# hall-lab/svtyper

Hardware: AMD Instinct MI355X
Metric: breakpoints genotyped/sec (higher is better)
Workload: dtype f64

## Files before the change

include/svtyper_reads.h:

```cpp
#ifndef SVTYPER_READS_H
#define SVTYPER_READS_H

#include <stdint.h>

#include "svtyper_hip.h"

#ifdef __cplusplus
extern "C" {
#endif

typedef struct svt_bam svt_bam;

int svt_bam_open(const char* path, svt_bam** out);
void svt_bam_close(svt_bam* bam);

int32_t svt_bam_n_references(const svt_bam* bam);
const char* svt_bam_reference_name(const svt_bam* bam, int32_t tid);
int64_t svt_bam_reference_length(const svt_bam* bam, int32_t tid);
int32_t svt_bam_tid(const svt_bam* bam, const char* name);
const char* svt_bam_header_text(const svt_bam* bam);

typedef struct svt_fetch_unit {
    int32_t tid_a, lo_a, hi_a;
    int32_t tid_b, lo_b, hi_b;
// ... 43 lines not shown
#define SVT_WALK_SA_CAP 6
#define SVT_WALK_NO_RG 7
#define SVT_WALK_UNKNOWN_RG 8
#define SVT_WALK_MALFORMED 9
#define SVT_WALK_MAPQ 10
#define SVT_WALK_N_REASONS 11

#define SVT_WALK_CAP_READS 0
#define SVT_WALK_CAP_NAME 1
#define SVT_WALK_CAP_CIGAR 2
#define SVT_WALK_CAP_SA_ENTRIES 3
#define SVT_WALK_CAP_SA_BYTES 4
#define SVT_WALK_CAP_RECORD 5
#define SVT_WALK_CAP_READS_LDS 6
uint32_t svt_evidence_walk_capacity(int which);

int svt_bam_evidence_walk_host(const svt_bam* bam, const svt_summarise_args* args, const svt_evidence_params* geometry,
                               svt_evidence* out, uint8_t* out_of_envelope, uint32_t* kept_reads);

typedef struct svt_evidence_device_stats {
    uint64_t n_units;
    uint64_t reads_walked;
    uint64_t units_skipped;
    uint64_t units_host;
    uint64_t units_host_by_reason[SVT_WALK_N_REASONS];
    uint64_t n_records;
    uint64_t bytes_uploaded;
    double host_arena_s;
    double upload_s;
    double device_walk_s;
// ... 100 lines not shown
```

svtyper_amd/csrc/svt_entry_evidence.h:

```cpp

static int run_inflate_kernel(const uint8_t* d_src, uint64_t src_len, const inf::Member* d_members, uint64_t n, uint8_t* d_dst, uint64_t dst_len,
                              uint32_t* d_status, std::vector<uint32_t>& status, hipStream_t s)
{
    status.assign(n, 0);
    constexpr uint64_t kGrid = 1u << 30;
    for (uint64_t at = 0; at < n; at += kGrid) {
        const uint64_t m = std::min(kGrid, n - at);
        hipLaunchKernelGGL(svt_inflate_kernel, dim3((unsigned)m), dim3(kInflateBlock), 0, s, d_src, src_len, d_members + at, (uint32_t)m, d_dst, dst_len,
                           d_status + at);
        HIP_TRY(hipGetLastError());
    }
    if (n) HIP_TRY(hipMemcpyAsync(status.data(), d_status, n * sizeof(uint32_t), hipMemcpyDeviceToHost, s));
    HIP_TRY(hipStreamSynchronize(s));
    return SVT_OK;
}

static thread_local svt_evidence_deep_stats g_deep_stats{};

struct EvidenceRoute {
    svt_evidence_inflate_stats* inflate_stats = nullptr;
    bool count_host_blocks = false;
    bool device_inflate() const { return inflate_stats != nullptr; }
};

struct EvidenceCall : CallStream {
    const svt_bam* const bam;
    const svt_summarise_args* const args;
    const svt_evidence_params* const geometry;
    const svt_evidence_batch* const header;
    const int device;
    const unsigned flags;
    const EvidenceRoute route;
    svt_evidence_device_stats& S;
    svt_evidence_deep_stats& DS = g_deep_stats;
    const uint64_t n = args->n_units;
    Pooled d_arena{device}, d_records{device}, d_compressed{device};
    DevScratch d_members, d_member_status;
    DevScratch d_ranges, d_units, d_windows, d_bps, d_rgs, d_refs, d_blob, d_flank, d_status, d_rows, d_reads, d_off, d_src, d_src_off, d_dst_off;
    DevScratch d_deep_unit, d_deep_status, d_deep_rows, d_deep_workspace;

    ew::Arena arena;
    ew::OpenPlan plan;
    EvidenceArgs a{};
    EvidenceDeepArgs da{};
    static constexpr size_t kLds = sizeof(ew::UnitScratch);
    std::vector<uint32_t> status, rows, reads;
    std::vector<uint32_t> deep_unit;
    uint32_t n_deep = 0, deep_grid = 0;
    std::vector<uint64_t> host_ids, host_counts;
    std::vector<svt_record> host_records;
    std::vector<uint8_t> host_skipped;
    std::vector<uint64_t> rec_offset;
    std::vector<svt_unit> units;
// ... 37 lines not shown
                svt_evidence_inflate_stats& I = *route.inflate_stats;
                SVT_TRY(d_compressed.get(plan.compressed_bytes + 8));
                for (const auto& sp : plan.spans) SVT_TRY(st.copy(static_cast<uint8_t*>(d_compressed.p) + sp.at, plan.file + sp.file_off, sp.bytes));
                SVT_TRY(upload(d_members, plan.members, st));
                SVT_TRY(d_member_status.alloc(plan.members.size() * sizeof(uint32_t)));
                SVT_TRY(st.finish());
                I.compressed_upload_s = since(t0);
                const auto t_kernel = now();
                std::vector<uint32_t> member_status;
                SVT_TRY(run_inflate_kernel(static_cast<const uint8_t*>(d_compressed.p), plan.compressed_bytes, d_members.as<inf::Member>(), plan.members.size(),
                                           static_cast<uint8_t*>(d_arena.p), plan.arena_bytes, d_member_status.as<uint32_t>(), member_status, s));
                I.inflate_kernel_s = since(t_kernel);
                I.blocks_failed = ew::apply_member_status(plan, member_status, arena);
            } else SVT_TRY(st.copy(d_arena.p, arena.bytes.data(), arena.bytes.size()));
            SVT_TRY(upload(d_ranges, arena.ranges, st));
            SVT_TRY(upload(d_units, arena.units, st));
            SVT_TRY(d_windows.alloc(n * sizeof(svt_fetch_unit)));
            SVT_TRY(st.copy(d_windows.p, args->windows, n * sizeof(svt_fetch_unit)));
            SVT_TRY(d_bps.alloc(n * sizeof(svt_breakpoint)));
            SVT_TRY(st.copy(d_bps.p, args->breakpoints, n * sizeof(svt_breakpoint)));
            SVT_TRY(upload(d_rgs, arena.rgs, st));
            SVT_TRY(upload(d_refs, arena.refs, st));
            SVT_TRY(upload(d_blob, arena.blob, st));
            SVT_TRY(upload(d_flank, flank, st));
            SVT_TRY(st.finish());
            S.bytes_uploaded = (route.device_inflate() ? plan.compressed_bytes + plan.members.size() * sizeof(inf::Member) : arena.bytes.size()) + arena.ranges.size() * sizeof(ew::Range) + n * (sizeof(ew::UnitRanges) + sizeof(svt_fetch_unit) + sizeof(svt_breakpoint)) + arena.blob.size();
        }
        SVT_TRY(d_status.alloc(n * sizeof(uint32_t)));
        SVT_TRY(d_rows.alloc(n * sizeof(uint32_t)));
        SVT_TRY(d_reads.alloc(n * sizeof(uint32_t)));
        SVT_TRY(d_off.alloc((n + 1) * sizeof(uint64_t)));
        HIP_TRY(hipStreamSynchronize(s));
        S.upload_s = since(t0);
        return SVT_OK;
    }
    int bind_arguments()
    {
        a.P = arena.params(args, geometry);
        a.P.arena = static_cast<const uint8_t*>(d_arena.p);
        a.P.ranges = d_ranges.as<ew::Range>();
        a.P.units = d_units.as<ew::UnitRanges>();
        a.P.windows = d_windows.as<svt_fetch_unit>();
        a.P.bps = d_bps.as<svt_breakpoint>();
        a.P.rgs = d_rgs.as<ew::NameRef>();
        a.P.refs = d_refs.as<ew::NameRef>();
        a.P.blob = d_blob.as<uint8_t>();
        a.P.lib_flank = d_flank.as<double>();
        a.n_units = (uint32_t)n;
        a.status = d_status.as<uint32_t>();
        a.n_rows = d_rows.as<uint32_t>();
        a.n_reads = d_reads.as<uint32_t>();
        a.rec_offset = d_off.as<uint64_t>();
        a.records = nullptr;
        static_assert(sizeof(ew::UnitScratch) <= 80 * 1024, "two workgroups of the evidence kernel per CU");
        static_assert(sizeof(ew::DeepScratch) <= 64 * 1024, "the deep kernel's static LDS");
// ... 253 lines not shown
```

svtyper_amd/csrc/svt_evidence_arena.h:

```cpp
#ifndef SVT_EVIDENCE_ARENA_H
#define SVT_EVIDENCE_ARENA_H

#include <cstdint>
#include <string>
#include <vector>

#include "svt_evidence_walk.h"
#include "svt_inflate.h"

namespace svt {
namespace ew {

struct Arena {
    std::vector<uint8_t> bytes;
    std::vector<Range> ranges;
    std::vector<UnitRanges> units;
    std::vector<NameRef> rgs, refs;
    std::vector<uint8_t> blob;
    uint64_t records_in_ranges = 0;
    uint64_t blocks = 0;
    double build_s = 0.0;
    bool open_ranges = false;
    Params params(const svt_summarise_args* args, const svt_evidence_params* geometry) const
    {
        Params P{};
        P.arena = bytes.data();
        P.arena_len = bytes.size();
        P.ranges = ranges.data();
        P.units = units.data();
        P.windows = args->windows;
        P.bps = args->breakpoints;
        P.rgs = rgs.data();
        P.refs = refs.data();
        P.blob = blob.data();
        P.lib_flank = geometry->lib_flank;
        P.n_rgs = (uint32_t)rgs.size();
        P.n_refs = (uint32_t)refs.size();
        P.n_libs = geometry->n_libs;
        P.min_aligned = geometry->min_aligned;
        P.split_slop = geometry->split_slop;
        P.count_mode = args->count_mode;
        P.max_reads = args->max_reads;
        P.open_ranges = open_ranges ? 1u : 0u;
        return P;
    }
};

inline bool deep_tier_unit(uint32_t status, uint32_t n_reads) { return status == EW_READS && n_reads <= kMaxReadsDeep; }


int build_arena(const svt_bam* bam, const svt_summarise_args* args, const svt_evidence_params* geometry, Arena& out);

struct OpenPlan {
    struct Span { uint64_t file_off, bytes, at; };
    const uint8_t* file = nullptr;
    uint64_t file_size = 0;
    std::vector<Span> spans;
    uint64_t compressed_bytes = 0;
    uint64_t arena_bytes = 0;
    std::vector<inf::Member> members;
    std::vector<std::pair<uint32_t, uint32_t>> range_members;
    double index_s = 0.0;
};

int build_arena_open(const svt_bam* bam, const svt_summarise_args* args, const svt_evidence_params* geometry, Arena& out, OpenPlan& plan);
void inflate_open_host(const OpenPlan& plan, Arena& out, unsigned n_threads, std::vector<uint32_t>& status);
// ... 12 lines not shown
```

svtyper_amd/csrc/svt_evidence_kernel.h:

```cpp
#ifndef SVT_EVIDENCE_KERNEL_H
#define SVT_EVIDENCE_KERNEL_H

#include "svt_evidence_walk.h"

namespace svt {

constexpr int kEvidenceBlock = 256;

struct EvidenceDevCtx {
    static __device__ __forceinline__ uint32_t lane() { return threadIdx.x; }
    static __device__ __forceinline__ uint32_t lanes() { return kEvidenceBlock; }
    static __device__ __forceinline__ void sync() { __syncthreads(); }
};

struct EvidenceArgs {
    ew::Params P;
    uint32_t n_units;
    uint32_t* status;
    uint32_t* n_rows;
    uint32_t* n_reads;
    const uint64_t* rec_offset;
    uint4* records;
};

// ... 64 lines not shown
```

svtyper_amd/csrc/svt_evidence_walk.h:

```cpp
#ifndef SVT_EVIDENCE_WALK_H
#define SVT_EVIDENCE_WALK_H

#include <stdint.h>

#include "../../include/svtyper_reads.h"
#include "svt_geometry_math.h"
#include "svt_record_rules.h"

namespace svt {
namespace ew {

using namespace rr;

constexpr uint32_t kMaxReads = 1024;
constexpr uint32_t kMaxReadsDeep = 16384;
constexpr uint32_t kSortTile = 2048;
constexpr uint32_t kMaxName = 128;
constexpr uint32_t kMaxCigar = 256;
constexpr uint32_t kMaxSaEntries = 8;
constexpr uint32_t kMaxSaBytes = 1024;
constexpr uint32_t kMaxRecord = 1u << 16;
constexpr uint32_t kBatch = 256;

enum : uint32_t {
    EW_OK = 0,
    EW_SKIPPED = 1,
    EW_RANGE = 2,
    EW_READS = 3,
    EW_NAME = 4,
    EW_CIGAR = 5,
    EW_SA_CAP = 6,
    EW_NO_RG = 7,
    EW_UNKNOWN_RG = 8,
    EW_MALFORMED = 9,
    EW_MAPQ = 10,
    EW_N_STATUS = 11
};

struct Range { uint32_t begin, end; };
struct UnitRanges { uint32_t first; uint16_t n[2]; uint32_t preset; };
struct NameRef { uint32_t off, len; int32_t value; };

struct Params {
    const uint8_t* arena;
    uint64_t arena_len;
    const Range* ranges;
    const UnitRanges* units;
    const svt_fetch_unit* windows;
    const svt_breakpoint* bps;
    const NameRef* rgs;
    const NameRef* refs;
    const uint8_t* blob;
    const double* lib_flank;
    uint32_t n_rgs, n_refs, n_libs;
    int32_t min_aligned, split_slop;
    int32_t count_mode;
    int64_t max_reads;
    uint32_t open_ranges;
};

struct ReadSum {
// ... 59 lines not shown
constexpr uint64_t kDeepSliceBytes = (uint64_t)kMaxReadsDeep * (sizeof(ReadSum) + sizeof(uint64_t) + 3 * sizeof(uint32_t));
static_assert(sizeof(ReadSum) == 52 && kDeepSliceBytes == 1179648, "1 179 648 bytes per slice");
SVT_HD Tables<uint32_t> deep_tables(uint8_t* slice)
{
    Tables<uint32_t> T;
    T.reads = reinterpret_cast<ReadSum*>(slice);
    T.key = reinterpret_cast<uint64_t*>(slice + (uint64_t)kMaxReadsDeep * sizeof(ReadSum));
    T.order = reinterpret_cast<uint32_t*>(T.key + kMaxReadsDeep);
    T.rows = T.order + kMaxReadsDeep;
    T.rowoff = T.rows + kMaxReadsDeep;
    T.cap = kMaxReadsDeep;
    return T;
}

struct HostCtx {
    static SVT_HD uint32_t lane() { return 0; }
    static SVT_HD uint32_t lanes() { return 1; }
    static SVT_HD void sync() {}
};

SVT_HD bool bytes_eq(const uint8_t* a, const uint8_t* b, uint32_t n)
{
    for (uint32_t i = 0; i < n; ++i) if (a[i] != b[i]) return false;
    return true;
}
SVT_HD int name_cmp(const uint8_t* a, uint32_t na, const uint8_t* b, uint32_t nb)
{
    const uint32_t n = na < nb ? na : nb;
    for (uint32_t i = 0; i < n; ++i) if (a[i] != b[i]) return a[i] < b[i] ? -1 : 1;
    return na < nb ? -1 : na > nb ? 1 : 0;
// ... 48 lines not shown
    if (r.tid >= 0 && (uint32_t)r.tid < P.n_refs) {
        const NameRef& nr = P.refs[r.tid];
        same_chrom = nr.len == fl[0] && bytes_eq(P.blob + nr.off, sa + fo[0], fl[0]);
    }
    const bool b_rev = fl[2] == 1 && sa[fo[2]] == '-';
    const Piece pa = {r.tid, r.pos, r.end, a_rev, query_pos(a, a_rev)};
    const Piece pb = {b_at < 0 ? -3 : b_at, mate_pos1 - 1, mate_pos1 - 1 + b.ref, b_rev, query_pos(b, b_rev)};
    bool self_left;
    if (!split_valid(pa, pb, same_chrom, left_clipped(a), self_left)) return EW_OK;
    rs.o_tid = pb.tid; rs.o_start = clip32(pb.start); rs.o_end = clip32(pb.end); rs.o_mapq = (uint8_t)mate_mapq;
    rs.bits |= (uint8_t)(RS_SPLIT | (b_rev ? RS_O_REV : 0) | (self_left ? RS_SELF_LEFT : 0));
    return EW_OK;
}

struct Eval { bool ovl, counted, keep; uint32_t early, late; };
SVT_HD void eval_record(const Params& P, const uint8_t* d, uint32_t size, uint32_t arena_off, int32_t wtid, int64_t lo, int64_t hi,
                        int64_t near_a, int64_t near_b, Eval& e, ReadSum& rs)
{
    e.ovl = e.counted = e.keep = false;
    e.early = e.late = EW_OK;
    Core r;
    if (!decode_core(d, size, r) || r.l_seq < 0 || r.tid != wtid || (int64_t)r.pos >= hi) { e.ovl = true; e.early = EW_RANGE; return; }
    int64_t rend = r.end;
    if (r.n_cigar == 0 || rend <= r.pos) rend = (int64_t)r.pos + 1;
    if (!(rend > lo)) return;
    e.ovl = true;
    e.counted = !(r.flag & (0x4 | 0x100 | 0x200 | 0x400));
    if (r.flag & (0x4 | 0x400)) return;
    Tags t;
    tags_begin(t);
    uint32_t tags_at = r.tags_off;
    const bool tags_ok = walk_tags(d, size, tags_at, false, t) == TAGS_END;
    if (!t.have_rg) { e.early = EW_NO_RG; return; }
    const int32_t at = find_name(P.rgs, P.n_rgs, P.blob, d + t.rg_off, t.rg_len);
    if (at < 0) { e.early = EW_UNKNOWN_RG; return; }
    const int32_t lib = P.rgs[at].value;
    if (lib < 0) return;
    e.keep = true;
    if (!tags_ok) { e.late = EW_MALFORMED; return; }
    if ((uint32_t)lib >= P.n_libs || lib > 0xffff) { e.late = EW_UNKNOWN_RG; return; }
    const uint32_t name_len = r.l_name ? r.l_name - 1 : 0;
// ... 9 lines not shown
    rs.flag = (uint16_t)r.flag;
    rs.lib = (uint16_t)lib;
    rs.mapq = (uint8_t)r.mapq;
    rs.o_mapq = 0;
    rs.bits = (uint8_t)((r.flag & 0x10) ? RS_REV : 0);
    if (r.flag & (0x100 | 0x800)) return;
    Intervals iv;
    aligned_intervals(d + 32 + r.l_name, r.n_cigar, r.pos, near_a, near_b, iv);
    rs.iv_s[0] = clip32(iv.s[0]); rs.iv_e[0] = clip32(iv.e[0]);
    rs.iv_s[1] = clip32(iv.s[1]); rs.iv_e[1] = clip32(iv.e[1]);
    rs.bits |= (uint8_t)iv.n;
    e.late = split_candidate(P, d, r, t, rs);
}

template <class X, class SC>
SVT_HD void gather_window(const Params& P, SC& S, const Tables<typename SC::Idx>& T, const Range* ranges, uint32_t n_ranges, int32_t wtid, int64_t lo, int64_t hi,
                          int64_t near_a, int64_t near_b)
{
    const uint32_t lane = X::lane(), lanes = X::lanes();
    const bool mode1 = P.count_mode == 1 && P.max_reads >= 0, mode0 = P.count_mode == 0 && P.max_reads >= 0;
    typedef Tables<typename SC::Idx> Tb;
    if (lo < 0) lo = 0;
    X::sync();
    if (lane == 0) { S.n_ovl = 0; S.n_counted = 0; S.window_done = 0; }
    for (uint32_t ri = 0; ri < n_ranges; ++ri) {
        const Range rg = ranges[ri];
        X::sync();
        if (S.window_done) break;
        if (lane == 0) {
            S.pos = rg.begin;
            S.range_done = 0;
            if (rg.end < rg.begin || (uint64_t)rg.end > P.arena_len) { if (S.status == EW_OK) S.status = EW_RANGE; }
        }
        X::sync();
        while (S.status == EW_OK && !S.range_done) {
            X::sync();
            if (lane == 0) {
                uint32_t nb = 0, pos = S.pos;
                while (nb < kBatch && pos < rg.end) {
                    if ((uint64_t)pos + 4 > rg.end) { S.status = EW_RANGE; break; }
                    const uint32_t size = ld32(P.arena + pos);
                    if (size < 32 || size > kMaxRecord || (uint64_t)pos + 4 + size > rg.end) { S.status = EW_RANGE; break; }
                    if (P.open_ranges && ((int32_t)ld32(P.arena + pos + 4) != wtid || (int64_t)(int32_t)ld32(P.arena + pos + 8) >= hi)) { S.window_done = 1; break; }
                    S.b.off[nb] = pos + 4;
                    S.b.size[nb] = size;
                    ++nb;
                    pos += 4 + size;
                }
                S.nb = nb;
                S.pos = pos;
                S.n_walked += nb;
                if (pos >= rg.end || nb == 0 || S.window_done) S.range_done = 1;
            }
            X::sync();
            if (S.status != EW_OK) break;
            const uint32_t nb = S.nb;
            for (uint32_t k = lane; k < nb; k += lanes) {
                Eval e;
                eval_record(P, P.arena + S.b.off[k], S.b.size[k], S.b.off[k], wtid, lo, hi, near_a, near_b, e, S.b.rs[k]);
                S.b.ovl[k] = e.ovl;
                S.b.counted[k] = e.counted;
                S.b.keep[k] = e.keep;
                S.b.ev[k] = (uint8_t)(e.early | (e.late << 4));
            }
            X::sync();
            if (lane == 0) {
                uint32_t n_ovl = S.n_ovl, n_counted = S.n_counted, n_reads = S.n_reads, st = EW_OK;
                for (uint32_t k = 0; k < nb && st == EW_OK; ++k) {
                    S.b.slot[k] = Tb::kNoSlot;
                    if (!S.b.ovl[k]) continue;
                    const int64_t i = (int64_t)n_ovl++;
                    const uint32_t early = S.b.ev[k] & 0xF, late = S.b.ev[k] >> 4;
                    if (early == EW_RANGE) { st = EW_RANGE; break; }
                    if (mode1 && S.b.counted[k] && (int64_t)++n_counted > P.max_reads) { st = EW_SKIPPED; break; }
                    if (early != EW_OK) { st = early; break; }
                    if (!S.b.keep[k]) continue;
                    if (mode0 && i > P.max_reads) { st = EW_SKIPPED; break; }
                    if (late != EW_OK) { st = late; break; }
                    if (n_reads < T.cap) S.b.slot[k] = (typename SC::Idx)n_reads;
                    ++n_reads;
                }
                S.n_ovl = n_ovl;
                S.n_counted = n_counted;
                S.n_reads = n_reads;
                if (st != EW_OK) S.status = st;
            }
            X::sync();
            if (S.status != EW_OK) break;
            for (uint32_t k = lane; k < nb; k += lanes)
                if (S.b.slot[k] != Tb::kNoSlot) T.reads[S.b.slot[k]] = S.b.rs[k];
            X::sync();
        }
        X::sync();
        if (S.status != EW_OK) return;
    }
}

SVT_HD ReadS absent_read() { ReadS r; r.tid = -1; r.start = r.end = r.iv0s = r.iv1s = r.iv0e = r.iv1e = 0; r.mapq = r.flags = r.extra = 0; return r; }
SVT_HD PieceS absent_piece() { PieceS p; p.tid = p.start = p.end = 0; p.mapq = p.flags = 0; return p; }
SVT_HD ReadS read_of_sum(const ReadSum& s)
{
    ReadS r;
    r.tid = s.tid; r.start = s.start; r.end = s.end;
    r.iv0s = s.iv_s[0]; r.iv1s = s.iv_s[1]; r.iv0e = s.iv_e[0]; r.iv1e = s.iv_e[1];
    r.mapq = s.mapq;
// ... 115 lines not shown
        X::sync();
    }
}

template <class X, class SC>
SVT_HD void walk_unit(const Params& P, uint64_t u, SC& S, const Tables<typename SC::Idx>& T, Record4* out)
{
    typedef typename SC::Idx Idx;
    typedef Tables<Idx> Tb;
    const uint32_t lane = X::lane(), lanes = X::lanes();
    const UnitRanges ur = P.units[u];
    const svt_fetch_unit w = P.windows[u];
    const svt_breakpoint bp = P.bps[u];
    if (lane == 0) { S.n_reads = 0; S.n_walked = 0; S.n_rows = 0; S.status = ur.preset; S.lcp = 0; }
    X::sync();
    if (S.status == EW_OK) gather_window<X>(P, S, T, P.ranges + ur.first, ur.n[0], w.tid_a, w.lo_a, w.hi_a, bp.pos_a, bp.pos_b);
    X::sync();
    if (S.status == EW_OK) gather_window<X>(P, S, T, P.ranges + ur.first + ur.n[0], ur.n[1], w.tid_b, w.lo_b, w.hi_b, bp.pos_a, bp.pos_b);
    X::sync();
    if (lane == 0 && S.status == EW_OK && S.n_reads > T.cap) S.status = EW_READS;
    X::sync();
    if (S.status != EW_OK) return;
    const uint32_t n = S.n_reads;
    if (n == 0) return;

    {
        uint32_t lcp = T.reads[0].name_len;
        const uint8_t* a = P.arena + T.reads[0].name_off;
        for (uint32_t k = lane; k < n; k += lanes) {
            const uint8_t* b = P.arena + T.reads[k].name_off;
            const uint32_t m = lcp < T.reads[k].name_len ? lcp : T.reads[k].name_len;
            uint32_t i = 0;
            while (i < m && a[i] == b[i]) ++i;
// ... 102 lines not shown
```

svtyper_amd/csrc/svt_reads.cpp:

```cpp

#include <dlfcn.h>
#include <fcntl.h>
#include <sys/mman.h>
#include <sys/stat.h>
#include <time.h>
#include <unistd.h>
#include <zlib.h>

#include <algorithm>
#include <atomic>
#include <chrono>
#include <condition_variable>
#include <cstdint>
#include <cstdio>
#include <cstdlib>
#include <cstring>
#include <map>
#include <memory>
#include <mutex>
#include <set>
#include <string>
#include <thread>
#include <unordered_map>
#include <vector>
// ... 1016 lines not shown
    if (args->n_units >= 0xFFFFFFF0ull) return fail(SVT_ERR_INVALID, "too many units in one call (< 2^32)");
    return SVT_OK;
}

void arena_names(const svt_bam* bam, const svt_summarise_args* args, Arena& out)
{
    auto add_name = [&](std::vector<NameRef>& tab, const char* p, size_t len, int32_t value) {
        tab.push_back(NameRef{(uint32_t)out.blob.size(), (uint32_t)len, value});
        out.blob.insert(out.blob.end(), p, p + len);
    };
    for (uint32_t i = 0; i < args->n_read_groups; ++i) add_name(out.rgs, args->read_groups[i], std::strlen(args->read_groups[i]), args->read_group_lib[i]);
    for (size_t i = 0; i < bam->ref_names.size(); ++i) add_name(out.refs, bam->ref_names[i].data(), bam->ref_names[i].size(), (int32_t)i);
    out.blob.resize(out.blob.size() + 8, 0);
}

struct RawRange { uint64_t first, last; uint32_t uoff, end_in_last; };
struct UnitRaw { uint64_t at = 0; unsigned worker = 0; uint16_t n[2] = {0, 0}; uint32_t preset = EW_OK; };
struct UnitPlan { std::vector<UnitRaw> units; std::vector<std::vector<RawRange>> ranges; };

enum : unsigned { kChunkRange = 1, kChunkLast = 2, kChunkHost = 4 };

template <typename Worker, typename Route>
int plan_units(const svt_bam* bam, const svt_summarise_args* args, unsigned nt, Route& route, UnitPlan& plan)
{
    const uint64_t n = args->n_units;
    plan.units.assign(n, UnitRaw());
    plan.ranges.assign(nt, std::vector<RawRange>());
    std::atomic<uint64_t> next(0);
    std::atomic<int> first_rc(SVT_OK);
    run_threads(nt, [&](unsigned t) {
        Worker worker(route, t);
// ... 3 lines not shown
            const uint64_t u0 = next.fetch_add(16);
            if (u0 >= n) return;
            for (uint64_t u = u0; u < std::min(n, u0 + 16); ++u) {
                UnitRaw& U = plan.units[u];
                U.at = list.size();
                U.worker = t;
                const svt_fetch_unit& w = args->windows[u];
                const int32_t tids[2] = {w.tid_a, w.tid_b};
                const int64_t los[2] = {w.lo_a, w.lo_b}, his[2] = {w.hi_a, w.hi_b};
                if (args->breakpoints[u].svtype > SVT_SVTYPE_BND) U.preset = EW_RANGE;
                for (int s = 0; s < 2 && U.preset == EW_OK; ++s) {
                    if (tids[s] < 0 || tids[s] >= (int32_t)bam->ref_names.size()) { U.preset = EW_RANGE; break; }
                    const int64_t beg = std::max<int64_t>(los[s], 0), end = his[s];
                    if (end <= beg) continue;
                    for (const auto& c : fetch_chunks(*bam, tids[s], beg, end)) {
                        RawRange r{0, 0, 0, 0};
                        const unsigned got = worker.chunk(tids[s], end, c.first, c.second, r);
                        if ((got & kChunkHost) || ((got & kChunkRange) && U.n[s] == 0xFFFF)) { U.preset = EW_RANGE; break; }
                        if (got & kChunkRange) { list.push_back(r); ++U.n[s]; }
                        if (got & kChunkLast) break;
                    }
                }
                if (U.preset != EW_OK) {
                    list.resize(U.at);
                    U.n[0] = U.n[1] = 0;
                }
            }
        }
    });
    if (first_rc.load() != SVT_OK) return fail(first_rc.load(), "cannot set up the inflate state");
    return SVT_OK;
// ... 8 lines not shown
        for (const RawRange& r : list) needs.push_back(Need{r.first, r.last});
    std::sort(needs.begin(), needs.end(), [](const Need& a, const Need& b) { return a.first < b.first; });
    for (size_t i = 0; i < needs.size();) {
        uint64_t last = needs[i].last;
        size_t j = i + 1;
        while (j < needs.size() && needs[j].first <= last) { last = std::max(last, needs[j].last); ++j; }
        if (const int rc = place(needs[i].first, last)) return rc;
        i = j;
    }
    return SVT_OK;
}

struct Placed { uint64_t at; uint32_t nth; };

void finish_ranges(UnitPlan& plan, const std::unordered_map<uint64_t, Placed>& placed, Arena& out,
                   std::vector<std::pair<uint32_t, uint32_t>>* range_members)
{
    const uint64_t n = plan.units.size();
    out.units.resize(n);
    for (uint64_t u = 0; u < n; ++u) {
        UnitRaw& U = plan.units[u];
        const RawRange* list = plan.ranges[U.worker].data() + U.at;
        const uint64_t nr = (uint64_t)U.n[0] + U.n[1];
        const size_t mark = out.ranges.size();
        for (uint64_t k = 0; k < nr; ++k) {
            const RawRange& r = list[k];
            const auto f = placed.find(r.first), l = placed.find(r.last);
            if (f == placed.end() || l == placed.end()) { U.preset = EW_RANGE; break; }
            const uint64_t begin = f->second.at + r.uoff, end = l->second.at + r.end_in_last;
            if (end > kArenaLimit) { U.preset = EW_RANGE; break; }
            out.ranges.push_back(Range{(uint32_t)std::min(begin, end), (uint32_t)end});
            if (range_members) range_members->emplace_back(f->second.nth, l->second.nth);
        }
        if (U.preset != EW_OK) {
            out.ranges.resize(mark);
            if (range_members) range_members->resize(mark);
            U.n[0] = U.n[1] = 0;
        }
        out.units[u] = UnitRanges{(uint32_t)mark, {U.n[0], U.n[1]}, U.preset};
    }
    out.ranges.push_back(Range{0, 0});
}

struct HostRoute {
    const svt_bam* bam;
    SharedBlocks shared_blocks;
    std::vector<std::vector<std::pair<uint64_t, BlockRef>>> touched;
    std::vector<uint64_t> n_records;
    HostRoute(const svt_bam* b, unsigned nt) : bam(b), touched(nt), n_records(nt, 0) {}
};
struct HostWorker {
    Bgzf z;
    std::vector<uint8_t> buf;
    uint64_t& n_records;
    HostWorker(HostRoute& route, unsigned t) : z(route.bam->file, &route.shared_blocks), n_records(route.n_records[t]) { z.touched = &route.touched[t]; }
    bool ok() const { return z.ok(); }
    unsigned chunk(int32_t tid, int64_t end, uint64_t vbeg, uint64_t vend, RawRange& r)
    {
        unsigned got = 0;
        z.seek(vbeg);
        while (z.tell() < vend) {
            const uint64_t at = z.tell();
            const bool beyond_block = z.offset_in_empty_block();
            uint32_t size = 0;
            const uint8_t* d = next_record(z, buf, size);
            if (!d) {
                if (z.failed() || z.tell() != at) got |= kChunkHost;
                break;
            }
            if ((int32_t)ld32(d) != tid || (int64_t)(int32_t)ld32(d + 4) >= end) { got |= kChunkLast; break; }
            if (!(got & kChunkRange)) {
                r.first = at >> 16;
                r.uoff = (uint32_t)(at & 0xFFFF);
                got |= kChunkRange;
                if (beyond_block) got |= kChunkHost;
            }
            z.last_read(&r.last, &r.end_in_last);
            ++n_records;
        }
        if (z.failed()) got |= kChunkHost;
        return got;
    }
};

struct OpenWorker {
    const OpenPlan& f;
    OpenWorker(OpenPlan& plan, unsigned) : f(plan) {}
    bool ok() const { return true; }
    unsigned chunk(int32_t, int64_t, uint64_t vbeg, uint64_t vend, RawRange& r) const
    {
        if (vend <= vbeg) return 0;
        const uint64_t cb = vbeg >> 16, ce = vend >> 16;
        const uint32_t ub = (uint32_t)(vbeg & 0xFFFF), ue = (uint32_t)(vend & 0xFFFF);
// ... 7 lines not shown
                break;
            }
            if (!inf::member_at(f.file, f.file_size, coff, src, clen, isize, next)) return kChunkHost;
            if (coff == cb && ub > isize) return kChunkHost;
            r.last = coff;
            r.end_in_last = isize;
            if (coff == ce) { r.end_in_last = std::min(ue, isize); break; }
            if (next > ce) return kChunkHost;
            if (next == ce && ue == 0) break;
            coff = next;
        }
        return kChunkRange;
    }
};

}

int build_arena(const svt_bam* bam, const svt_summarise_args* args, const svt_evidence_params* geometry, Arena& out)
{
    if (const int rc = check_arena_args(bam, args, geometry)) return rc;
    const auto t_begin = std::chrono::steady_clock::now();
    out = Arena();
    arena_names(bam, args, out);
    const unsigned nt = arena_threads(args, args->n_units);
    const std::unique_ptr<HostRoute> route(new HostRoute(bam, nt));
    UnitPlan plan;
    if (const int rc = plan_units<HostWorker>(bam, args, nt, *route, plan)) return rc;

    std::unordered_map<uint64_t, BlockRef> blocks;
    for (auto& log : route->touched) {
        for (auto& e : log) blocks.emplace(e.first, e.second);
// ... 14 lines not shown
        }
    });
    out.bytes.resize(std::min<uint64_t>(total, kArenaLimit) + 8);
    {
        std::atomic<size_t> at(0);
        run_threads(std::min<unsigned>(nt, 16u), [&](unsigned) {
            for (;;) {
                const size_t k = at.fetch_add(8);
                if (k >= copies.size()) return;
                for (size_t c = k; c < std::min(copies.size(), k + 8); ++c)
                    if (copies[c].at + copies[c].b->data.size() <= kArenaLimit && !copies[c].b->data.empty())
                        std::memcpy(out.bytes.data() + copies[c].at, copies[c].b->data.data(), copies[c].b->data.size());
            }
        });
    }
    finish_ranges(plan, placed, out, nullptr);
    for (uint64_t c : route->n_records) out.records_in_ranges += c;
    out.blocks = copies.size();
    out.build_s = std::chrono::duration<double>(std::chrono::steady_clock::now() - t_begin).count();
    return SVT_OK;
}

int build_arena_open(const svt_bam* bam, const svt_summarise_args* args, const svt_evidence_params* geometry, Arena& out, OpenPlan& plan)
{
    if (const int rc = check_arena_args(bam, args, geometry)) return rc;
    const auto t_begin = std::chrono::steady_clock::now();
    out = Arena();
    out.open_ranges = true;
    plan = OpenPlan();
    plan.file = bam->file.data;
    plan.file_size = bam->file.size;
// ... 13 lines not shown
                placed[coff] = Placed{total, (uint32_t)plan.members.size()};
                plan.members.push_back(inf::Member{span.at + (src - span.file_off), clen, isize, total});
                span.bytes = next - span.file_off;
            }
            total += isize;
            if (coff == last) break;
            coff = next;
        }
        if (span.bytes) { plan.spans.push_back(span); plan.compressed_bytes += span.bytes; }
        return (int)SVT_OK;
    });
    if (rc) return rc;
    plan.arena_bytes = plan.members.empty() ? 0 : plan.members.back().dst + plan.members.back().isize;
    out.bytes.resize(plan.arena_bytes + 8);
    out.blocks = plan.members.size();
    finish_ranges(units, placed, out, &plan.range_members);
    plan.index_s = out.build_s = std::chrono::duration<double>(std::chrono::steady_clock::now() - t_begin).count();
    return SVT_OK;
}

void inflate_open_host(const OpenPlan& plan, Arena& out, unsigned n_threads, std::vector<uint32_t>& status)
{
    const size_t m = plan.members.size();
    status.assign(m, inf::INF_OK);
    std::atomic<size_t> next(0);
    run_threads(std::max(1u, std::min<unsigned>(n_threads, (unsigned)std::max<size_t>(m, 1))), [&](unsigned) {
        std::unique_ptr<inf::Scratch> S(new inf::Scratch());
        for (;;) {
            const size_t k0 = next.fetch_add(8);
            if (k0 >= m) return;
            for (size_t k = k0; k < std::min(m, k0 + 8); ++k) {
// ... 502 lines not shown
{
    return guarded([&]() -> int {
        if (n && (!status || (!out && out_off && out_off[n]))) return fail(SVT_ERR_INVALID, "null argument");
        std::vector<svt::inf::Member> members(n);
        if (const int rc = svt::ew::bgzf_members(data, len, block_off, n, out_off, members.data())) return rc;
        std::unique_ptr<svt::inf::Scratch> S(new svt::inf::Scratch());
        for (uint64_t k = 0; k < n; ++k) {
            const svt::inf::Member& m = members[k];
            status[k] = m.isize == svt::inf::kNoMember ? (uint32_t)svt::inf::INF_MEMBER
                                                       : svt::inf::inflate_member<svt::inf::HostCtx>(data + m.src, m.clen, out + m.dst, m.isize, *S);
        }
        return SVT_OK;
    });
}

uint32_t svt_evidence_walk_capacity(int which)
{
    switch (which) {
    case SVT_WALK_CAP_READS: return svt::ew::kMaxReadsDeep;
    case SVT_WALK_CAP_READS_LDS: return svt::ew::kMaxReads;
    case SVT_WALK_CAP_NAME: return svt::ew::kMaxName;
    case SVT_WALK_CAP_CIGAR: return svt::ew::kMaxCigar;
    case SVT_WALK_CAP_SA_ENTRIES: return svt::ew::kMaxSaEntries;
    case SVT_WALK_CAP_SA_BYTES: return svt::ew::kMaxSaBytes;
    case SVT_WALK_CAP_RECORD: return svt::ew::kMaxRecord;
    default: return 0;
    }
}

static int svt_bam_scan_library_impl(const svt_bam* bam, uint32_t n_read_groups, const char* const* read_groups, int64_t num_samp,
// ... 489 lines not shown
```

Before: 3.447 billion.

## Parallelise evidence range walk with host-recorded record checkpoints

Result: no change. 3.423 billion (-0.7%).

```diff
diff --git a/include/svtyper_reads.h b/include/svtyper_reads.h
--- a/include/svtyper_reads.h
+++ b/include/svtyper_reads.h
@@ -81,6 +81,7 @@
 #define SVT_WALK_CAP_RECORD 5
 #define SVT_WALK_CAP_READS_LDS 6
 uint32_t svt_evidence_walk_capacity(int which);
+int svt_debug_walk_checkpoints(int on);
 
 int svt_bam_evidence_walk_host(const svt_bam* bam, const svt_summarise_args* args, const svt_evidence_params* geometry,
                                svt_evidence* out, uint8_t* out_of_envelope, uint32_t* kept_reads);
diff --git a/svtyper_amd/csrc/svt_entry_evidence.h b/svtyper_amd/csrc/svt_entry_evidence.h
--- a/svtyper_amd/csrc/svt_entry_evidence.h
+++ b/svtyper_amd/csrc/svt_entry_evidence.h
@@ -36,7 +36,7 @@
     const uint64_t n = args->n_units;
     Pooled d_arena{device}, d_records{device}, d_compressed{device};
     DevScratch d_members, d_member_status;
-    DevScratch d_ranges, d_units, d_windows, d_bps, d_rgs, d_refs, d_blob, d_flank, d_status, d_rows, d_reads, d_off, d_src, d_src_off, d_dst_off;
+    DevScratch d_ranges, d_range_cps, d_checkpoints, d_units, d_windows, d_bps, d_rgs, d_refs, d_blob, d_flank, d_status, d_rows, d_reads, d_off, d_src, d_src_off, d_dst_off;
     DevScratch d_deep_unit, d_deep_status, d_deep_rows, d_deep_workspace;
 
     ew::Arena arena;
@@ -104,6 +104,10 @@
                 I.blocks_failed = ew::apply_member_status(plan, member_status, arena);
             } else SVT_TRY(st.copy(d_arena.p, arena.bytes.data(), arena.bytes.size()));
             SVT_TRY(upload(d_ranges, arena.ranges, st));
+            if (!arena.range_cps.empty()) {
+                SVT_TRY(upload(d_range_cps, arena.range_cps, st));
+                SVT_TRY(upload(d_checkpoints, arena.checkpoints, st));
+            }
             SVT_TRY(upload(d_units, arena.units, st));
             SVT_TRY(d_windows.alloc(n * sizeof(svt_fetch_unit)));
             SVT_TRY(st.copy(d_windows.p, args->windows, n * sizeof(svt_fetch_unit)));
@@ -114,7 +118,7 @@
             SVT_TRY(upload(d_blob, arena.blob, st));
             SVT_TRY(upload(d_flank, flank, st));
             SVT_TRY(st.finish());
-            S.bytes_uploaded = (route.device_inflate() ? plan.compressed_bytes + plan.members.size() * sizeof(inf::Member) : arena.bytes.size()) + arena.ranges.size() * sizeof(ew::Range) + n * (sizeof(ew::UnitRanges) + sizeof(svt_fetch_unit) + sizeof(svt_breakpoint)) + arena.blob.size();
+            S.bytes_uploaded = (route.device_inflate() ? plan.compressed_bytes + plan.members.size() * sizeof(inf::Member) : arena.bytes.size()) + arena.ranges.size() * sizeof(ew::Range) + arena.range_cps.size() * sizeof(ew::RangeCheckpoints) + (arena.range_cps.empty() ? 0 : arena.checkpoints.size() * sizeof(uint32_t)) + n * (sizeof(ew::UnitRanges) + sizeof(svt_fetch_unit) + sizeof(svt_breakpoint)) + arena.blob.size();
         }
         SVT_TRY(d_status.alloc(n * sizeof(uint32_t)));
         SVT_TRY(d_rows.alloc(n * sizeof(uint32_t)));
@@ -129,6 +133,8 @@
         a.P = arena.params(args, geometry);
         a.P.arena = static_cast<const uint8_t*>(d_arena.p);
         a.P.ranges = d_ranges.as<ew::Range>();
+        a.P.range_cps = arena.range_cps.empty() ? nullptr : d_range_cps.as<ew::RangeCheckpoints>();
+        a.P.checkpoints = arena.range_cps.empty() ? nullptr : d_checkpoints.as<uint32_t>();
         a.P.units = d_units.as<ew::UnitRanges>();
         a.P.windows = d_windows.as<svt_fetch_unit>();
         a.P.bps = d_bps.as<svt_breakpoint>();
diff --git a/svtyper_amd/csrc/svt_evidence_arena.h b/svtyper_amd/csrc/svt_evidence_arena.h
--- a/svtyper_amd/csrc/svt_evidence_arena.h
+++ b/svtyper_amd/csrc/svt_evidence_arena.h
@@ -14,6 +14,8 @@
 struct Arena {
     std::vector<uint8_t> bytes;
     std::vector<Range> ranges;
+    std::vector<RangeCheckpoints> range_cps;
+    std::vector<uint32_t> checkpoints;
     std::vector<UnitRanges> units;
     std::vector<NameRef> rgs, refs;
     std::vector<uint8_t> blob;
@@ -27,6 +29,8 @@
         P.arena = bytes.data();
         P.arena_len = bytes.size();
         P.ranges = ranges.data();
+        P.range_cps = range_cps.empty() ? nullptr : range_cps.data();
+        P.checkpoints = checkpoints.data();
         P.units = units.data();
         P.windows = args->windows;
         P.bps = args->breakpoints;
@@ -50,6 +54,7 @@
 
 
 int build_arena(const svt_bam* bam, const svt_summarise_args* args, const svt_evidence_params* geometry, Arena& out);
+bool walk_checkpoints(bool on);
 
 struct OpenPlan {
     struct Span { uint64_t file_off, bytes, at; };
diff --git a/svtyper_amd/csrc/svt_evidence_kernel.h b/svtyper_amd/csrc/svt_evidence_kernel.h
--- a/svtyper_amd/csrc/svt_evidence_kernel.h
+++ b/svtyper_amd/csrc/svt_evidence_kernel.h
@@ -8,6 +8,7 @@
 constexpr int kEvidenceBlock = 256;
 
 struct EvidenceDevCtx {
+    static constexpr uint32_t kLanes = kEvidenceBlock;
     static __device__ __forceinline__ uint32_t lane() { return threadIdx.x; }
     static __device__ __forceinline__ uint32_t lanes() { return kEvidenceBlock; }
     static __device__ __forceinline__ void sync() { __syncthreads(); }
diff --git a/svtyper_amd/csrc/svt_evidence_walk.h b/svtyper_amd/csrc/svt_evidence_walk.h
--- a/svtyper_amd/csrc/svt_evidence_walk.h
+++ b/svtyper_amd/csrc/svt_evidence_walk.h
@@ -21,6 +21,8 @@
 constexpr uint32_t kMaxSaBytes = 1024;
 constexpr uint32_t kMaxRecord = 1u << 16;
 constexpr uint32_t kBatch = 256;
+constexpr uint32_t kCheckpointEvery = 64;
+static_assert(kCheckpointEvery <= 64 && kBatch % kCheckpointEvery == 0, "a segment's overlap verdicts are bits of 64-bit words; whole segments make up a batch");
 
 enum : uint32_t {
     EW_OK = 0,
@@ -38,6 +40,7 @@
 };
 
 struct Range { uint32_t begin, end; };
+struct RangeCheckpoints { uint32_t first, count; };
 struct UnitRanges { uint32_t first; uint16_t n[2]; uint32_t preset; };
 struct NameRef { uint32_t off, len; int32_t value; };
 
@@ -45,6 +48,8 @@
     const uint8_t* arena;
     uint64_t arena_len;
     const Range* ranges;
+    const RangeCheckpoints* range_cps;
+    const uint32_t* checkpoints;
     const UnitRanges* units;
     const svt_fetch_unit* windows;
     const svt_breakpoint* bps;
@@ -134,6 +139,7 @@
 }
 
 struct HostCtx {
+    static constexpr uint32_t kLanes = 1;
     static SVT_HD uint32_t lane() { return 0; }
     static SVT_HD uint32_t lanes() { return 1; }
     static SVT_HD void sync() {}
@@ -212,17 +218,24 @@
 }
 
 struct Eval { bool ovl, counted, keep; uint32_t early, late; };
+SVT_HD bool record_overlaps(const uint8_t* d, uint32_t size, int32_t wtid, int64_t lo, int64_t hi, Core& r, bool& bad)
+{
+    bad = !decode_core(d, size, r) || r.l_seq < 0 || r.tid != wtid || (int64_t)r.pos >= hi;
+    if (bad) return true;
+    int64_t rend = r.end;
+    if (r.n_cigar == 0 || rend <= r.pos) rend = (int64_t)r.pos + 1;
+    return rend > lo;
+}
 SVT_HD void eval_record(const Params& P, const uint8_t* d, uint32_t size, uint32_t arena_off, int32_t wtid, int64_t lo, int64_t hi,
                         int64_t near_a, int64_t near_b, Eval& e, ReadSum& rs)
 {
     e.ovl = e.counted = e.keep = false;
     e.early = e.late = EW_OK;
     Core r;
-    if (!decode_core(d, size, r) || r.l_seq < 0 || r.tid != wtid || (int64_t)r.pos >= hi) { e.ovl = true; e.early = EW_RANGE; return; }
-    int64_t rend = r.end;
-    if (r.n_cigar == 0 || rend <= r.pos) rend = (int64_t)r.pos + 1;
-    if (!(rend > lo)) return;
+    bool bad;
+    if (!record_overlaps(d, size, wtid, lo, hi, r, bad)) return;
     e.ovl = true;
+    if (bad) { e.early = EW_RANGE; return; }
     e.counted = !(r.flag & (0x4 | 0x100 | 0x200 | 0x400));
     if (r.flag & (0x4 | 0x400)) return;
     Tags t;
@@ -262,12 +275,149 @@
 }
 
 template <class X, class SC>
-SVT_HD void gather_window(const Params& P, SC& S, const Tables<typename SC::Idx>& T, const Range* ranges, uint32_t n_ranges, int32_t wtid, int64_t lo, int64_t hi,
-                          int64_t near_a, int64_t near_b)
-{
+SVT_HD void eval_staged(const Params& P, SC& S, uint32_t nb, int32_t wtid, int64_t lo, int64_t hi, int64_t near_a, int64_t near_b)
+{
+    for (uint32_t k = X::lane(); k < nb; k += X::lanes()) {
+        Eval e;
+        eval_record(P, P.arena + S.b.off[k], S.b.size[k], S.b.off[k], wtid, lo, hi, near_a, near_b, e, S.b.rs[k]);
+        S.b.ovl[k] = e.ovl;
+        S.b.counted[k] = e.counted;
+        S.b.keep[k] = e.keep;
+        S.b.ev[k] = (uint8_t)(e.early | (e.late << 4));
+    }
+}
+template <class SC>
+SVT_HD uint32_t book_staged(const Params& P, SC& S, const Tables<typename SC::Idx>& T, uint32_t nb)
+{
+    typedef Tables<typename SC::Idx> Tb;
+    const bool mode1 = P.count_mode == 1 && P.max_reads >= 0, mode0 = P.count_mode == 0 && P.max_reads >= 0;
+    uint32_t n_ovl = S.n_ovl, n_counted = S.n_counted, n_reads = S.n_reads, st = EW_OK, k = 0;
+    for (; k < nb; ++k) {
+        S.b.slot[k] = Tb::kNoSlot;
+        if (!S.b.ovl[k]) continue;
+        const int64_t i = (int64_t)n_ovl++;
+        const uint32_t early = S.b.ev[k] & 0xF, late = S.b.ev[k] >> 4;
+        if (early == EW_RANGE) { st = EW_RANGE; break; }
+        if (mode1 && S.b.counted[k] && (int64_t)++n_counted > P.max_reads) { st = EW_SKIPPED; break; }
+        if (early != EW_OK) { st = early; break; }
+        if (!S.b.keep[k]) continue;
+        if (mode0 && i > P.max_reads) { st = EW_SKIPPED; break; }
+        if (late != EW_OK) { st = late; break; }
+        if (n_reads < T.cap) S.b.slot[k] = (typename SC::Idx)n_reads;
+        ++n_reads;
+    }
+    S.n_ovl = n_ovl;
+    S.n_counted = n_counted;
+    S.n_reads = n_reads;
+    if (st != EW_OK) S.status = st;
+    return k;
+}
+template <class X, class SC>
+SVT_HD void store_staged(SC& S, const Tables<typename SC::Idx>& T, uint32_t nb)
+{
+    for (uint32_t k = X::lane(); k < nb; k += X::lanes())
+        if (S.b.slot[k] != Tables<typename SC::Idx>::kNoSlot) T.reads[S.b.slot[k]] = S.b.rs[k];
+}
+
+constexpr uint32_t kSegEnd = 1, kSegStop = 2, kSegBad = 3;
+template <class X, class SC>
+SVT_HD void gather_range_checkpoints(const Params& P, SC& S, const Tables<typename SC::Idx>& T, const Range rg, const uint32_t* cp, uint32_t n_cp,
+                                     int32_t wtid, int64_t lo, int64_t hi, int64_t near_a, int64_t near_b)
+{
+    constexpr uint32_t kStride = X::kLanes * kCheckpointEvery >= kBatch ? 1u : kBatch / (kCheckpointEvery * X::kLanes);
+    constexpr uint32_t kSeg = kCheckpointEvery * kStride, kWords = (kSeg + 63) / 64;
+    static_assert(X::kLanes <= kBatch && kBatch % kSeg == 0 && (X::kLanes * kSeg) % kBatch == 0 && kSeg <= 0x3ff, "a word of the staging area per lane; passes of whole batches");
     const uint32_t lane = X::lane(), lanes = X::lanes();
-    const bool mode1 = P.count_mode == 1 && P.max_reads >= 0, mode0 = P.count_mode == 0 && P.max_reads >= 0;
-    typedef Tables<typename SC::Idx> Tb;
+    const uint32_t n_seg = (n_cp + kStride - 1) / kStride;
+    for (uint32_t s0 = 0; s0 < n_seg; s0 += lanes) {
+        X::sync();
+        if (S.status != EW_OK) return;
+        const uint32_t seg = s0 + lane;
+        uint64_t mask[kWords];
+        for (uint32_t w = 0; w < kWords; ++w) mask[w] = 0;
+        uint32_t n = 0, how = kSegEnd, pos0 = 0, mine = 0;
+        if (seg < n_seg) {
+            pos0 = cp[(uint64_t)seg * kStride];
+            uint32_t pos = pos0;
+            how = 0;
+            while (n < kSeg && pos < rg.end) {
+                if ((uint64_t)pos + 4 > rg.end) { how = kSegBad; break; }
+                const uint32_t size = ld32(P.arena + pos);
+                if (size < 32 || size > kMaxRecord || (uint64_t)pos + 4 + size > rg.end) { how = kSegBad; break; }
+                const uint8_t* d = P.arena + pos + 4;
+                const int64_t rpos = (int64_t)(int32_t)ld32(d + 4);
+                if (P.open_ranges && ((int32_t)ld32(d) != wtid || rpos >= hi)) { how = kSegStop; break; }
+                Core r;
+                bool bad;
+                if (rpos >= lo || record_overlaps(d, size, wtid, lo, hi, r, bad)) {
+                    mask[kWords == 1 ? 0 : n >> 6] |= 1ull << (n & 63);
+                    ++mine;
+                }
+                ++n;
+                pos += 4 + size;
+            }
+            if (how == 0 && pos >= rg.end) how = kSegEnd;
+            else if (how == 0 && seg == n_seg - 1) how = kSegBad;
+        }
+        S.b.cnt[lane] = mine | (n << 10) | (how << 20);
+        X::sync();
+        uint32_t t = lanes;
+        for (uint32_t k = lanes; k-- > 0;)
+            if (S.b.cnt[k] >> 20) t = k;
+        const uint32_t t_how = t < lanes ? S.b.cnt[t] >> 20 : 0u;
+        const uint32_t pass_records = t < lanes ? t * kSeg + ((S.b.cnt[t] >> 10) & 0x3ff) : lanes * kSeg;
+        const uint32_t looked_at = t_how == kSegBad ? pass_records / kBatch * kBatch : pass_records;
+        uint32_t before = 0, total = 0;
+        for (uint32_t k = 0; k < lanes && k * kSeg < looked_at; ++k) {
+            const uint32_t c = S.b.cnt[k] & 0x3ff;
+            before += k < lane ? c : 0u;
+            total += c;
+        }
+        if (!(lane * kSeg < looked_at)) mine = 0;
+        uint32_t q = before, cur = pos0, j = 0;
+        const uint32_t q_end = before + mine;
+        for (uint32_t r0 = 0; r0 < total; r0 += kBatch) {
+            const uint32_t r1 = total - r0 < kBatch ? total : r0 + kBatch, nb = r1 - r0;
+            while (q < q_end && q < r1 && j < n) {
+                const uint32_t size = ld32(P.arena + cur);
+                if ((mask[kWords == 1 ? 0 : j >> 6] >> (j & 63)) & 1) {
+                    S.b.off[q - r0] = cur + 4;
+                    S.b.size[q - r0] = size;
+                    S.b.idx[q - r0] = lane * kSeg + j;
+                    ++q;
+                }
+                cur += 4 + size;
+                ++j;
+            }
+            X::sync();
+            eval_staged<X>(P, S, nb, wtid, lo, hi, near_a, near_b);
+            X::sync();
+            if (lane == 0) {
+                const uint32_t k = book_staged(P, S, T, nb);
+                if (k < nb) {
+                    const uint32_t batch_end = (S.b.idx[k] / kBatch + 1) * kBatch;
+                    S.n_walked += batch_end < pass_records ? batch_end : pass_records;
+                }
+            }
+            X::sync();
+            if (S.status != EW_OK) return;
+            store_staged<X>(S, T, nb);
+            X::sync();
+        }
+        if (lane == 0) {
+            S.n_walked += pass_records;
+            if (t_how == kSegBad) S.status = EW_RANGE;
+            if (t_how == kSegStop) S.window_done = 1;
+        }
+        if (t < lanes) return;
+    }
+}
+
+template <class X, class SC>
+SVT_HD void gather_window(const Params& P, SC& S, const Tables<typename SC::Idx>& T, const Range* ranges, const RangeCheckpoints* cps, uint32_t n_ranges,
+                          int32_t wtid, int64_t lo, int64_t hi, int64_t near_a, int64_t near_b)
+{
+    const uint32_t lane = X::lane();
     if (lo < 0) lo = 0;
     X::sync();
     if (lane == 0) { S.n_ovl = 0; S.n_counted = 0; S.window_done = 0; }
@@ -281,7 +431,8 @@
             if (rg.end < rg.begin || (uint64_t)rg.end > P.arena_len) { if (S.status == EW_OK) S.status = EW_RANGE; }
         }
         X::sync();
-        while (S.status == EW_OK && !S.range_done) {
+        if (cps && cps[ri].count) gather_range_checkpoints<X>(P, S, T, rg, P.checkpoints + cps[ri].first, cps[ri].count, wtid, lo, hi, near_a, near_b);
+        else while (S.status == EW_OK && !S.range_done) {
             X::sync();
             if (lane == 0) {
                 uint32_t nb = 0, pos = S.pos;
@@ -303,40 +454,12 @@
             X::sync();
             if (S.status != EW_OK) break;
             const uint32_t nb = S.nb;
-            for (uint32_t k = lane; k < nb; k += lanes) {
-                Eval e;
-                eval_record(P, P.arena + S.b.off[k], S.b.size[k], S.b.off[k], wtid, lo, hi, near_a, near_b, e, S.b.rs[k]);
-                S.b.ovl[k] = e.ovl;
-                S.b.counted[k] = e.counted;
-                S.b.keep[k] = e.keep;
-                S.b.ev[k] = (uint8_t)(e.early | (e.late << 4));
-            }
-            X::sync();
-            if (lane == 0) {
-                uint32_t n_ovl = S.n_ovl, n_counted = S.n_counted, n_reads = S.n_reads, st = EW_OK;
-                for (uint32_t k = 0; k < nb && st == EW_OK; ++k) {
-                    S.b.slot[k] = Tb::kNoSlot;
-                    if (!S.b.ovl[k]) continue;
-                    const int64_t i = (int64_t)n_ovl++;
-                    const uint32_t early = S.b.ev[k] & 0xF, late = S.b.ev[k] >> 4;
-                    if (early == EW_RANGE) { st = EW_RANGE; break; }
-                    if (mode1 && S.b.counted[k] && (int64_t)++n_counted > P.max_reads) { st = EW_SKIPPED; break; }
-                    if (early != EW_OK) { st = early; break; }
-                    if (!S.b.keep[k]) continue;
-                    if (mode0 && i > P.max_reads) { st = EW_SKIPPED; break; }
-                    if (late != EW_OK) { st = late; break; }
-                    if (n_reads < T.cap) S.b.slot[k] = (typename SC::Idx)n_reads;
-                    ++n_reads;
-                }
-                S.n_ovl = n_ovl;
-                S.n_counted = n_counted;
-                S.n_reads = n_reads;
-                if (st != EW_OK) S.status = st;
-            }
+            eval_staged<X>(P, S, nb, wtid, lo, hi, near_a, near_b);
+            X::sync();
+            if (lane == 0) book_staged(P, S, T, nb);
             X::sync();
             if (S.status != EW_OK) break;
-            for (uint32_t k = lane; k < nb; k += lanes)
-                if (S.b.slot[k] != Tb::kNoSlot) T.reads[S.b.slot[k]] = S.b.rs[k];
+            store_staged<X>(S, T, nb);
             X::sync();
         }
         X::sync();
@@ -482,9 +605,9 @@
     const svt_breakpoint bp = P.bps[u];
     if (lane == 0) { S.n_reads = 0; S.n_walked = 0; S.n_rows = 0; S.status = ur.preset; S.lcp = 0; }
     X::sync();
-    if (S.status == EW_OK) gather_window<X>(P, S, T, P.ranges + ur.first, ur.n[0], w.tid_a, w.lo_a, w.hi_a, bp.pos_a, bp.pos_b);
-    X::sync();
-    if (S.status == EW_OK) gather_window<X>(P, S, T, P.ranges + ur.first + ur.n[0], ur.n[1], w.tid_b, w.lo_b, w.hi_b, bp.pos_a, bp.pos_b);
+    if (S.status == EW_OK) gather_window<X>(P, S, T, P.ranges + ur.first, P.range_cps ? P.range_cps + ur.first : nullptr, ur.n[0], w.tid_a, w.lo_a, w.hi_a, bp.pos_a, bp.pos_b);
+    X::sync();
+    if (S.status == EW_OK) gather_window<X>(P, S, T, P.ranges + ur.first + ur.n[0], P.range_cps ? P.range_cps + ur.first + ur.n[0] : nullptr, ur.n[1], w.tid_b, w.lo_b, w.hi_b, bp.pos_a, bp.pos_b);
     X::sync();
     if (lane == 0 && S.status == EW_OK && S.n_reads > T.cap) S.status = EW_READS;
     X::sync();
diff --git a/svtyper_amd/csrc/svt_reads.cpp b/svtyper_amd/csrc/svt_reads.cpp
--- a/svtyper_amd/csrc/svt_reads.cpp
+++ b/svtyper_amd/csrc/svt_reads.cpp
@@ -1054,7 +1054,7 @@
     out.blob.resize(out.blob.size() + 8, 0);
 }
 
-struct RawRange { uint64_t first, last; uint32_t uoff, end_in_last; };
+struct RawRange { uint64_t first, last; uint32_t uoff, end_in_last; uint64_t cp_at; uint32_t cp_n; };
 struct UnitRaw { uint64_t at = 0; unsigned worker = 0; uint16_t n[2] = {0, 0}; uint32_t preset = EW_OK; };
 struct UnitPlan { std::vector<UnitRaw> units; std::vector<std::vector<RawRange>> ranges; };
 
@@ -1088,7 +1088,7 @@
                     const int64_t beg = std::max<int64_t>(los[s], 0), end = his[s];
                     if (end <= beg) continue;
                     for (const auto& c : fetch_chunks(*bam, tids[s], beg, end)) {
-                        RawRange r{0, 0, 0, 0};
+                        RawRange r{0, 0, 0, 0, 0, 0};
                         const unsigned got = worker.chunk(tids[s], end, c.first, c.second, r);
                         if ((got & kChunkHost) || ((got & kChunkRange) && U.n[s] == 0xFFFF)) { U.preset = EW_RANGE; break; }
                         if (got & kChunkRange) { list.push_back(r); ++U.n[s]; }
@@ -1127,10 +1127,15 @@
 struct Placed { uint64_t at; uint32_t nth; };
 
 void finish_ranges(UnitPlan& plan, const std::unordered_map<uint64_t, Placed>& placed, Arena& out,
-                   std::vector<std::pair<uint32_t, uint32_t>>* range_members)
+                   std::vector<std::pair<uint32_t, uint32_t>>* range_members, const std::vector<std::vector<uint32_t>>* checkpoints)
 {
     const uint64_t n = plan.units.size();
     out.units.resize(n);
+    if (checkpoints) {
+        size_t total = 0;
+        for (const auto& list : *checkpoints) total += list.size();
+        out.checkpoints.reserve(total);
+    }
     for (uint64_t u = 0; u < n; ++u) {
         UnitRaw& U = plan.units[u];
         const RawRange* list = plan.ranges[U.worker].data() + U.at;
@@ -1144,15 +1149,24 @@
             if (end > kArenaLimit) { U.preset = EW_RANGE; break; }
             out.ranges.push_back(Range{(uint32_t)std::min(begin, end), (uint32_t)end});
             if (range_members) range_members->emplace_back(f->second.nth, l->second.nth);
+            if (checkpoints) {
+                const uint32_t have = begin <= end && out.checkpoints.size() + r.cp_n <= 0xFFFFFFFFull ? r.cp_n : 0;
+                out.range_cps.push_back(RangeCheckpoints{(uint32_t)out.checkpoints.size(), have});
+                const uint32_t* rel = (*checkpoints)[U.worker].data() + r.cp_at;
+                for (uint32_t c = 0; c < have; ++c) out.checkpoints.push_back((uint32_t)begin + rel[c]);
+            }
         }
         if (U.preset != EW_OK) {
             out.ranges.resize(mark);
             if (range_members) range_members->resize(mark);
+            if (checkpoints && out.range_cps.size() > mark) { out.checkpoints.resize(out.range_cps[mark].first); out.range_cps.resize(mark); }
             U.n[0] = U.n[1] = 0;
         }
         out.units[u] = UnitRanges{(uint32_t)mark, {U.n[0], U.n[1]}, U.preset};
     }
     out.ranges.push_back(Range{0, 0});
+    if (checkpoints) out.range_cps.push_back(RangeCheckpoints{(uint32_t)out.checkpoints.size(), 0});
+    out.checkpoints.push_back(0);
 }
 
 struct HostRoute {
@@ -1160,17 +1174,21 @@
     SharedBlocks shared_blocks;
     std::vector<std::vector<std::pair<uint64_t, BlockRef>>> touched;
     std::vector<uint64_t> n_records;
-    HostRoute(const svt_bam* b, unsigned nt) : bam(b), touched(nt), n_records(nt, 0) {}
+    std::vector<std::vector<uint32_t>> checkpoints;
+    HostRoute(const svt_bam* b, unsigned nt) : bam(b), touched(nt), n_records(nt, 0), checkpoints(nt) {}
 };
 struct HostWorker {
     Bgzf z;
     std::vector<uint8_t> buf;
     uint64_t& n_records;
-    HostWorker(HostRoute& route, unsigned t) : z(route.bam->file, &route.shared_blocks), n_records(route.n_records[t]) { z.touched = &route.touched[t]; }
+    std::vector<uint32_t>& checkpoints;
+    HostWorker(HostRoute& route, unsigned t) : z(route.bam->file, &route.shared_blocks), n_records(route.n_records[t]), checkpoints(route.checkpoints[t]) { z.touched = &route.touched[t]; }
     bool ok() const { return z.ok(); }
     unsigned chunk(int32_t tid, int64_t end, uint64_t vbeg, uint64_t vend, RawRange& r)
     {
         unsigned got = 0;
+        uint64_t rel = 0;
+        uint32_t in_segment = 0;
         z.seek(vbeg);
         while (z.tell() < vend) {
             const uint64_t at = z.tell();
@@ -1185,11 +1203,15 @@
             if (!(got & kChunkRange)) {
                 r.first = at >> 16;
                 r.uoff = (uint32_t)(at & 0xFFFF);
+                r.cp_at = checkpoints.size();
                 got |= kChunkRange;
                 if (beyond_block) got |= kChunkHost;
             }
             z.last_read(&r.last, &r.end_in_last);
             ++n_records;
+            if (in_segment == 0) { checkpoints.push_back((uint32_t)rel); ++r.cp_n; }
+            in_segment = in_segment + 1 == kCheckpointEvery ? 0 : in_segment + 1;
+            rel += 4 + (uint64_t)size;
         }
         if (z.failed()) got |= kChunkHost;
         return got;
@@ -1227,7 +1249,11 @@
     }
 };
 
-}
+std::atomic<bool> g_walk_checkpoints{std::getenv("SVT_NO_WALK_CHECKPOINTS") == nullptr};
+
+}
+
+bool walk_checkpoints(bool on) { return g_walk_checkpoints.exchange(on); }
 
 int build_arena(const svt_bam* bam, const svt_summarise_args* args, const svt_evidence_params* geometry, Arena& out)
 {
@@ -1272,7 +1298,7 @@
             }
         });
     }
-    finish_ranges(plan, placed, out, nullptr);
+    finish_ranges(plan, placed, out, nullptr, g_walk_checkpoints.load() ? &route->checkpoints : nullptr);
     for (uint64_t c : route->n_records) out.records_in_ranges += c;
     out.blocks = copies.size();
     out.build_s = std::chrono::duration<double>(std::chrono::steady_clock::now() - t_begin).count();
@@ -1316,7 +1342,7 @@
     plan.arena_bytes = plan.members.empty() ? 0 : plan.members.back().dst + plan.members.back().isize;
     out.bytes.resize(plan.arena_bytes + 8);
     out.blocks = plan.members.size();
-    finish_ranges(units, placed, out, &plan.range_members);
+    finish_ranges(units, placed, out, &plan.range_members, nullptr);
     plan.index_s = out.build_s = std::chrono::duration<double>(std::chrono::steady_clock::now() - t_begin).count();
     return SVT_OK;
 }
@@ -1849,6 +1875,8 @@
     });
 }
 
+int svt_debug_walk_checkpoints(int on) { return svt::ew::walk_checkpoints(on != 0) ? 1 : 0; }
+
 uint32_t svt_evidence_walk_capacity(int which)
 {
     switch (which) {
```
